# kazuto1011/dusty-gan-v2

Hardware: AMD Instinct MI355X
Metric: range-images/sec (G+D step) on dusty_v2 64x512 (higher is better)
Workload: dtype bf16; 1 GPU; configs[2]: configs/gans/dusty_v2.yaml full G+D train step (G step + D step + lazy R1 + ADA + EMA + Adam), 64x512 synthetic; global_batch=64, per_gpu_batch=64, parallelism=dp1, hip_graph=True, d_epilogue_dtype=fp32, pe_table_precomputed=True

## Files before the change

dusty-gan-v2_amd/csrc/api.hip:

```cpp
#include "common.h"

extern "C" int dgv2_abi_version(void) { return 48; }
```

dusty-gan-v2_amd/csrc/fir_mfma.hip:

```cpp
#include <type_traits>

#include "gemm_core.h"

namespace {

constexpr int FM_CT = 32;
constexpr int FM_CB = 32;
constexpr int FM_WIN = FM_CT + 16;
#ifndef DGV2_FIR_RS
#define DGV2_FIR_RS 8
#endif
constexpr int FM_RS = DGV2_FIR_RS;
constexpr int FM_RING = 2 * FM_RS;
static_assert(FM_RS == 8 || FM_RS == 4, "rows per step");
constexpr int FM_XBYTES = FM_RS * FM_WIN * 64;
constexpr int FM_ZROW = 2048 + 64;
constexpr int FM_ZBYTES = FM_RING * FM_ZROW;
constexpr int FM_YROW = 2048 + 16;
constexpr int FM_YBYTES = FM_RS * FM_YROW;
constexpr int FM_NLD = FM_RS * FM_WIN * 4 / 256;

struct FMGeom {
  int B, C, H, W, nt;
  const uint4* bands;
  const bf16_t* ref;
  float alpha, ascale;
  float* partial;
  uint8_t* y8;
};

struct FMTabs {
  int H, W, Eh, Ew;
  const int* idx_h; const float* coef_h; const int* cnt_h;
  const int* idx_w; const float* coef_w; const int* cnt_w;
  int* err;
};

typedef __attribute__((ext_vector_type(4))) unsigned fm_u32x4;
typedef __attribute__((address_space(3))) s16x4 fm_lds_s16x4;

__device__ __forceinline__ unsigned fm_pack2(float a, float b) {
  union { bf16_t h[2]; unsigned u; } p;
  p.h[0] = (bf16_t)a;
  p.h[1] = (bf16_t)b;
  return p.u;
}

__global__ __launch_bounds__(64) void fir_bands_kernel(uint4* __restrict__ bands, FMTabs t) {
  const int lane = threadIdx.x, li = lane & 15, kg = lane >> 4;
  const int nh = t.H / FM_RS + 1;
  float v[8];
#pragma unroll
  for (int j = 0; j < 8; ++j) v[j] = 0.f;
  bool bad = false;
  if ((int)blockIdx.x < nh) {
    const int s = blockIdx.x, ho = s * FM_RS - FM_RS / 2 + li;
    if (li < FM_RS && ho >= 0 && ho < t.H) {
      const int n = t.cnt_h[ho];
      for (int e = 0; e < n; ++e) {
        const int r = t.idx_h[ho * t.Eh + e];
        const float cf = t.coef_h[ho * t.Eh + e];
        if (r < s * FM_RS - FM_RS || r >= s * FM_RS + FM_RS || r < 0 || r >= t.H) bad = true;
#pragma unroll
        for (int j = 0; j < 8; ++j)
          if ((r & (FM_RING - 1)) == 8 * kg + j) v[j] += cf;
      }
    }
  } else {
    const int wt = blockIdx.x - nh, wo = 16 * wt + li;
    const int n = t.cnt_w[wo];
    for (int e = 0; e < n; ++e) {
      int rel = t.idx_w[wo * t.Ew + e] - (16 * wt - 8);
      rel = rel < 0 ? rel + t.W : (rel >= t.W ? rel - t.W : rel);
      const float cf = t.coef_w[wo * t.Ew + e];
      if ((unsigned)rel >= 32u) bad = true;
#pragma unroll
      for (int j = 0; j < 8; ++j)
        if (rel == 8 * kg + j) v[j] += cf;
    }
  }
#pragma unroll
  for (int j = 0; j < 8; ++j)
    if ((float)(bf16_t)v[j] != v[j]) bad = true;
  bands[(int64_t)blockIdx.x * 64 + lane] =
      make_uint4(fm_pack2(v[0], v[1]), fm_pack2(v[2], v[3]), fm_pack2(v[4], v[5]), fm_pack2(v[6], v[7]));
  if (bad) atomicOr(t.err, DGV2_STATUS_FIR_TABLE);
}

// ... 150 lines not shown
          bsum[j] += o.get(j);
        }
      }
      if constexpr (!ACT) {
        if (g.y8) {
          float f[8];
#pragma unroll
          for (int j = 0; j < 8; ++j) f[j] = o.get(j);
          *reinterpret_cast<uint2*>(g.y8 + off) = pack_fp8x8(f);
          continue;
        }
      }
      if (g.nt) o.store_nt(y + off);
      else o.store(y + off);
    }
    th = th_next;
  }

  if constexpr (ACT) {
    float* fold = reinterpret_cast<float*>(Xs);
    __syncthreads();
#pragma unroll
    for (int j = 0; j < 8; ++j) fold[tid * 8 + j] = bsum[j];
    __syncthreads();
    if (tid < FM_CB) {
      const int o8 = tid >> 3, j = tid & 7;
      float s2 = 0.f;
      for (int t = o8; t < 256; t += 4) s2 += fold[t * 8 + j];
      g.partial[((int64_t)b * gridDim.x + c0col / FM_CT) * g.C + cb0 + tid] = s2;
    }
  }
}

__global__ __launch_bounds__(256) void fm_bias_reduce_kernel(float* __restrict__ gb, const float* __restrict__ partial,
                                                             int nblk, int C) {
  __shared__ float red[16];
  const int c = blockIdx.x;
  float s = 0.f;
#pragma unroll 4
  for (int k = threadIdx.x; k < nblk; k += 256) s += partial[(int64_t)k * C + c];
  s = block_sum(s, red);
  if (threadIdx.x == 0) gb[c] = s;
}

bool fm_covers(int B, int C, int H, int W) {
  return B > 0 && C % FM_CB == 0 && H % FM_RS == 0 && H >= FM_RS && W % FM_CT == 0 && W >= FM_CT && B < 65536 &&
         C / FM_CB < 65536;
}

constexpr size_t FM_LDS = (size_t)FM_XBYTES + FM_ZBYTES + FM_YBYTES;

int64_t fm_band_bytes(int H, int W) { return 1024 * ((int64_t)H / FM_RS + 1 + W / 16); }

}

extern "C" int dgv2_fir_same_mfma_prep(void* bands, int64_t bands_bytes, int64_t* bytes_needed, const int* idx_h,
                                       const float* coef_h, const int* cnt_h, int Eh, const int* idx_w, const float* coef_w,
                                       const int* cnt_w, int Ew, int H, int W, int* status, void* stream) {
  if (H < FM_RS || H % FM_RS || W < FM_CT || W % FM_CT || Eh < 1 || Ew < 1) return DGV2_ENOTSUP;
  const int64_t need = fm_band_bytes(H, W);
  if (bytes_needed) *bytes_needed = need;
  if (!bands) return bytes_needed ? 0 : DGV2_EINVAL;
  if (bands_bytes < need || !aligned16(bands) || !idx_h || !coef_h || !cnt_h || !idx_w || !coef_w || !cnt_w) return DGV2_EINVAL;
  if (!status) return DGV2_EINVAL;
  FMTabs t{H, W, Eh, Ew, idx_h, coef_h, cnt_h, idx_w, coef_w, cnt_w, status};
  fir_bands_kernel<<<(int)(need / 1024), 64, 0, (hipStream_t)stream>>>((uint4*)bands, t);
  DGV2_RETURN_LAST();
}

extern "C" int dgv2_fir_same_mfma(void* y, const void* x, const void* bands, int B, int C, int H, int W, void* stream) {
  if (!y || !x || !bands) return DGV2_EINVAL;
  if (!fm_covers(B, C, H, W)) return DGV2_ENOTSUP;
  if (!aligned16(x) || !aligned16(y) || !aligned16(bands)) return DGV2_EINVAL;
  FMGeom g{B, C, H, W, nt_output((int64_t)B * H * W * C * 2) ? 1 : 0, (const uint4*)bands, nullptr, 1.f, 1.f, nullptr, nullptr};
  auto kern = fir_same_mfma_kernel<false>;
  if (FM_LDS > 64 * 1024) {
    hipError_t e = hipFuncSetAttribute((const void*)kern, hipFuncAttributeMaxDynamicSharedMemorySize, (int)FM_LDS);
    if (e != hipSuccess) return (int)e;
  }
  kern<<<dim3(W / FM_CT, C / FM_CB, B), 256, FM_LDS, (hipStream_t)stream>>>((bf16_t*)y, (const bf16_t*)x, g);
  DGV2_RETURN_LAST();
}

extern "C" int dgv2_fir_same_mfma_q8(void* y8, const void* x, const void* bands, int B, int C, int H, int W, void* stream) {
  if (!y8 || !x || !bands) return DGV2_EINVAL;
  if (!fm_covers(B, C, H, W)) return DGV2_ENOTSUP;
  if (!aligned16(x) || (reinterpret_cast<uintptr_t>(y8) & 7) || !aligned16(bands)) return DGV2_EINVAL;
  FMGeom g{B, C, H, W, 0, (const uint4*)bands, nullptr, 1.f, 1.f, nullptr, (uint8_t*)y8};
  auto kern = fir_same_mfma_kernel<false>;
  if (FM_LDS > 64 * 1024) {
    hipError_t e = hipFuncSetAttribute((const void*)kern, hipFuncAttributeMaxDynamicSharedMemorySize, (int)FM_LDS);
    if (e != hipSuccess) return (int)e;
  }
  kern<<<dim3(W / FM_CT, C / FM_CB, B), 256, FM_LDS, (hipStream_t)stream>>>((bf16_t*)nullptr, (const bf16_t*)x, g);
  DGV2_RETURN_LAST();
}

extern "C" int dgv2_fir_same_mfma_actbwd(void* y, float* gb, float* scratch, int64_t scratch_elems, int64_t* blocks_needed,
                                         const void* x, const void* ref, const void* bands, int B, int C, int H, int W,
                                         float alpha, float scale, void* stream) {
  if (!fm_covers(B, C, H, W)) return DGV2_ENOTSUP;
  const int64_t blocks = (int64_t)B * (W / FM_CT);
  if (blocks_needed) *blocks_needed = blocks;
  if (!scratch) return blocks_needed ? 0 : DGV2_EINVAL;
  if (!y || !gb || !x || !ref || !bands) return DGV2_EINVAL;
  if (scratch_elems < blocks * C || !aligned16(x) || !aligned16(y) || !aligned16(ref) || !aligned16(bands)) return DGV2_EINVAL;
  FMGeom g{B, C, H, W, 0, (const uint4*)bands, (const bf16_t*)ref, alpha, scale, scratch, nullptr};
  auto kern = fir_same_mfma_kernel<true>;
  if (FM_LDS > 64 * 1024) {
    hipError_t e = hipFuncSetAttribute((const void*)kern, hipFuncAttributeMaxDynamicSharedMemorySize, (int)FM_LDS);
    if (e != hipSuccess) return (int)e;
  }
  hipStream_t st = (hipStream_t)stream;
  kern<<<dim3(W / FM_CT, C / FM_CB, B), 256, FM_LDS, st>>>((bf16_t*)y, (const bf16_t*)x, g);
  fm_bias_reduce_kernel<<<C, 256, 0, st>>>(gb, scratch, (int)blocks, C);
  DGV2_RETURN_LAST();
}
```

dusty-gan-v2_amd/dgv2_native/__init__.py:

```python
import ctypes
import os

import torch

_HERE = os.path.dirname(os.path.abspath(__file__))
LIB_PATH = os.environ.get("DGV2_LIB_PATH") or os.path.join(os.path.dirname(_HERE), "lib", "libdgv2.so")

F32, BF16 = 0, 1
ABI_VERSION = 48

_c_int, _c_i64, _c_f32, _c_ptr = ctypes.c_int, ctypes.c_int64, ctypes.c_float, ctypes.c_void_p

SIGNATURES = {
    "dgv2_abi_version": [],
    "dgv2_fused_bias_act": [_c_ptr] * 4 + [_c_i64] * 3 + [_c_int, _c_int, _c_f32, _c_f32, _c_int, _c_ptr],
    "dgv2_bias_grad": [_c_ptr, _c_ptr, _c_i64, _c_i64, _c_i64, _c_int, _c_ptr],
    "dgv2_bias_act_bwd": [_c_ptr] * 4 + [_c_i64, _c_int, _c_f32, _c_f32, _c_ptr, _c_i64, _c_int, _c_ptr],
    "dgv2_bias_act_bwd_rs": [_c_ptr] * 4 + [_c_i64, _c_int, _c_f32, _c_f32, _c_ptr, _c_ptr, _c_i64, _c_int, _c_ptr],
    "dgv2_surface_normal": [_c_ptr, _c_ptr] + [_c_int] * 5 + [_c_ptr],
    "dgv2_mbstd_cat_fwd": [_c_ptr] * 3 + [_c_int] * 7 + [_c_ptr],
    "dgv2_mbstd_cat_bwd": [_c_ptr] * 3 + [_c_int] * 7 + [_c_ptr],
    "dgv2_gemm_x3": [_c_ptr, _c_ptr, _c_i64, _c_ptr, _c_ptr, _c_int, _c_int, _c_i64, _c_int, _c_int, _c_i64, _c_i64, _c_i64,
                     _c_int, _c_f32, _c_ptr],
    "dgv2_pe_wgrad_scratch": [_c_ptr] + [_c_int] * 4,
    "dgv2_pe_wgrad": [_c_ptr, _c_ptr, _c_i64, _c_ptr, _c_ptr] + [_c_int] * 4 + [_c_i64, _c_int, _c_ptr],
    "dgv2_mbstd_cat_fwd_x": [_c_ptr] * 3 + [_c_int] * 8 + [_c_ptr],
    "dgv2_mbstd_cat_bwd_x": [_c_ptr] * 3 + [_c_int] * 8 + [_c_ptr],
    "dgv2_scale_cast": [_c_ptr] * 3 + [_c_i64, _c_int, _c_int, _c_int, _c_ptr],
    "dgv2_upfirdn2d": [_c_ptr] * 3 + [_c_int] * 15 + [_c_ptr],
    "dgv2_resample": [_c_ptr] * 4 + [_c_int] * 19 + [_c_ptr],
    "dgv2_resample_tab": [_c_ptr] * 5 + [_c_int] + [_c_ptr] * 3 + [_c_int] * 10 + [_c_ptr],
    "dgv2_resample_tab_add": [_c_ptr] * 6 + [_c_int] + [_c_ptr] * 3 + [_c_int] * 8 + [_c_ptr],
    "dgv2_resample_tab_add_affine": [_c_ptr] * 8 + [_c_int] + [_c_ptr] * 3 + [_c_int] * 8 + [_c_ptr],
    "dgv2_fourier_feature": [_c_ptr] * 5 + [_c_int] * 8 + [_c_ptr],
    "dgv2_downsample_angle": [_c_ptr] * 4 + [_c_int] * 5 + [_c_ptr],
    "dgv2_bmm_nn": [_c_ptr] * 3 + [_c_int] * 6 + [_c_i64, _c_ptr, _c_int, _c_f32, _c_f32, _c_int, _c_int, _c_ptr],
    "dgv2_bmm_tn": [_c_ptr] * 3 + [_c_int] * 7 + [_c_ptr],
    "dgv2_bmm_nn_cat": [_c_ptr] * 4 + [_c_int] * 5 + [_c_ptr, _c_int, _c_f32, _c_f32, _c_int, _c_int, _c_ptr],
    "dgv2_bmm_nn_cat_sq": [_c_ptr] * 4 + [_c_int] * 5 + [_c_ptr, _c_ptr, _c_int, _c_f32, _c_f32, _c_int, _c_int, _c_ptr, _c_int, _c_ptr,
                           _c_ptr],
    "dgv2_bmm_nn_sq": [_c_ptr] * 3 + [_c_int] * 6 + [_c_i64, _c_ptr, _c_ptr, _c_int, _c_f32, _c_f32, _c_ptr, _c_int, _c_int, _c_ptr, _c_int,
                       _c_ptr, _c_ptr],
# ... 6 lines not shown
    "dgv2_kitti_project": [_c_ptr] * 4 + [_c_int] * 4 + [_c_f32, _c_f32, _c_int, _c_ptr],
    "dgv2_fps_scratch": [_c_ptr, _c_int, _c_int],
    "dgv2_fps": [_c_ptr] * 3 + [_c_int] * 3 + [_c_ptr],
    "dgv2_gather_points": [_c_ptr] * 3 + [_c_int] * 4 + [_c_ptr],
    "dgv2_gather_points_grad": [_c_ptr] * 3 + [_c_int] * 4 + [_c_ptr],
    "dgv2_chamfer_fwd": [_c_ptr] * 6 + [_c_int] * 3 + [_c_ptr],
    "dgv2_nn_search": [_c_ptr] * 4 + [_c_int] * 4 + [_c_ptr],
    "dgv2_chamfer_bwd": [_c_ptr] * 8 + [_c_int] * 3 + [_c_ptr],
    "dgv2_emd_approxmatch": [_c_ptr] * 4 + [_c_int] * 3 + [_c_ptr],
    "dgv2_emd_matchcost": [_c_ptr] * 4 + [_c_int] * 3 + [_c_ptr],
    "dgv2_emd_matchcost_grad": [_c_ptr] * 5 + [_c_int] * 3 + [_c_ptr],
    "dgv2_nsgan_loss": [_c_ptr, _c_ptr, _c_ptr, _c_int, _c_int, _c_f32, _c_ptr, _c_ptr, _c_ptr],
    "dgv2_modconv_pe_dgrad_actbwd": [_c_ptr, _c_ptr, _c_ptr, _c_i64] + [_c_ptr] * 5 + [_c_f32, _c_f32] + [_c_int] * 4 + [_c_ptr],
    "dgv2_colmean_lerp": [_c_ptr, _c_ptr, _c_int, _c_int, _c_i64, _c_f32, _c_ptr],
    "dgv2_d_tail_fwd": [_c_ptr] * 6 + [_c_int, _c_int] + [_c_f32] * 4 + [_c_ptr],
    "dgv2_d_tail_bwd": [_c_ptr] * 7 + [_c_int, _c_int] + [_c_f32] * 4 + [_c_ptr],
    "dgv2_rng_fill": [_c_ptr] * 5 + [_c_int, _c_ptr, _c_ptr],
    "dgv2_modconv_up_fwd": [_c_ptr] * 4 + [_c_int] * 7 + [_c_ptr] * 6 + [_c_int, _c_f32, _c_f32, _c_int, _c_ptr, _c_int, _c_ptr,
                            _c_ptr],
    "dgv2_modconv_up_t_lag": [_c_ptr] * 4 + [_c_f32] + [_c_ptr] * 4 + [_c_int] * 9 + [_c_ptr, _c_int, _c_ptr, _c_ptr],
    "dgv2_fir_same_mfma_q8": [_c_ptr] * 3 + [_c_int] * 4 + [_c_ptr],
    "dgv2_resample_tab_q8": [_c_ptr] * 5 + [_c_int] + [_c_ptr] * 3 + [_c_int] * 7 + [_c_ptr],
    "dgv2_fp8_quant_weights": [_c_ptr] * 6 + [_c_int] + [_c_ptr] * 3,
    "dgv2_fp8_dequant": [_c_ptr, _c_ptr, _c_i64, _c_f32, _c_ptr],
    "dgv2_conv_taps_fp8": [_c_ptr] * 4 + [_c_int] * 14 + [_c_ptr, _c_int, _c_ptr, _c_ptr, _c_int, _c_f32, _c_f32, _c_ptr],
    "dgv2_modconv_up_t": [_c_ptr] * 5 + [_c_f32] + [_c_int] * 9 + [_c_ptr],
    "dgv2_up2_lag_sumsq": [_c_ptr] * 5 + [_c_int] * 5 + [_c_ptr, _c_int, _c_ptr, _c_ptr],
    "dgv2_resample_tab_actbwd": [_c_ptr, _c_ptr, _c_ptr, _c_i64, _c_ptr, _c_ptr, _c_ptr] + [_c_ptr] * 3 + [_c_int] + [_c_ptr] * 3
                                + [_c_int] * 7 + [_c_f32, _c_f32, _c_int, _c_ptr],
    "dgv2_fir_same_mfma_prep": [_c_ptr, _c_i64, _c_ptr] + [_c_ptr] * 3 + [_c_int] + [_c_ptr] * 3 + [_c_int] * 3 + [_c_ptr, _c_ptr],
    "dgv2_fir_same_mfma": [_c_ptr] * 3 + [_c_int] * 4 + [_c_ptr],
    "dgv2_fir_same_mfma_actbwd": [_c_ptr, _c_ptr, _c_ptr, _c_i64, _c_ptr, _c_ptr, _c_ptr, _c_ptr] + [_c_int] * 4
                                 + [_c_f32, _c_f32, _c_ptr],
    "dgv2_resample_tab_sq": [_c_ptr] * 5 + [_c_int] + [_c_ptr] * 3 + [_c_int] * 10 + [_c_ptr, _c_int, _c_ptr, _c_ptr],
    "dgv2_bmm_tn_cat": [_c_ptr] * 4 + [_c_int] * 6 + [_c_ptr],
    "dgv2_lerp_list": [_c_ptr] * 3 + [_c_int, _c_f32, _c_ptr],
    "dgv2_adam_prep": [_c_ptr, _c_ptr, _c_f32, _c_f32, _c_ptr],
    "dgv2_adam_step": [_c_ptr] * 5 + [_c_int, _c_ptr] + [_c_f32] * 4 + [_c_ptr],
    "dgv2_pack2d": [_c_ptr] * 4 + [_c_int] * 3 + [_c_ptr],
    "dgv2_unpack2d": [_c_ptr] * 4 + [_c_int] * 3 + [_c_ptr],
    "dgv2_ema_scalar": [_c_ptr] * 3 + [_c_int] + [_c_f32] * 3 + [_c_int, _c_ptr, _c_int, _c_ptr],
    "dgv2_ema_scalar_group": [_c_ptr, _c_ptr, _c_int, _c_ptr, _c_int] + [_c_f32] * 3 + [_c_int, _c_ptr, _c_ptr],
    "dgv2_bmm_nn_small": [_c_ptr] * 4 + [_c_int] * 5 + [_c_ptr],
    "dgv2_bmm_nn_small_act": [_c_ptr] * 4 + [_c_int] * 4 + [_c_ptr, _c_ptr, _c_f32, _c_f32, _c_ptr, _c_ptr, _c_i64, _c_ptr, _c_int,
                              _c_ptr],
    "dgv2_bmm_tn_small": [_c_ptr] * 3 + [_c_int] * 5 + [_c_ptr],
    "dgv2_head_bwd": [_c_ptr] * 5 + [_c_i64] + [_c_ptr] * 7 + [_c_f32, _c_f32] + [_c_int] * 5 + [_c_ptr],
    "dgv2_transpose_list": [_c_ptr] * 5 + [_c_int] * 3 + [_c_ptr],
    "dgv2_mod_prep_all_fwd": [_c_ptr] * 13 + [_c_ptr, _c_int, _c_int, _c_ptr],
    "dgv2_mod_prep_all_bwd": [_c_ptr, _c_i64] + [_c_ptr] * 15 + [_c_ptr, _c_int, _c_int, _c_ptr, _c_i64, _c_ptr],
    "dgv2_mod_prep_all_bwd_scratch": [_c_ptr, _c_ptr, _c_ptr, _c_int, _c_int],
    "dgv2_mod_prep_fwd": [_c_ptr] * 8 + [_c_int] * 9 + [_c_ptr],
    "dgv2_mod_prep_bwd": [_c_ptr] * 11 + [_c_int] * 9 + [_c_ptr],
    "dgv2_sum_squares": [_c_ptr, _c_ptr, _c_i64, _c_int, _c_int, _c_int, _c_ptr],
    "dgv2_conv_fwd": [_c_ptr] * 3 + [_c_int] * 10 + [_c_ptr, _c_int, _c_f32, _c_f32, _c_int, _c_ptr],
    "dgv2_conv_taps": [_c_ptr] * 3 + [_c_int] * 17 + [_c_ptr] + [_c_int] * 3 + [_c_ptr, _c_ptr, _c_int, _c_f32, _c_f32, _c_int,
                                                                               _c_ptr],
    "dgv2_conv_taps_ex": [_c_ptr] * 3 + [_c_int] * 14 + [_c_ptr, _c_int, _c_int, _c_ptr, _c_int, _c_ptr] + [_c_int] * 3
    + [_c_ptr, _c_ptr, _c_int, _c_f32, _c_f32, _c_int, _c_ptr],
    "dgv2_conv_taps_ld": [_c_ptr, _c_int, _c_ptr, _c_ptr] + [_c_int] * 14 + [_c_ptr, _c_int, _c_int, _c_ptr, _c_int, _c_ptr] + [_c_int] * 3
    + [_c_ptr, _c_ptr, _c_int, _c_f32, _c_f32, _c_int, _c_ptr],
    "dgv2_conv_wgrad_direct": [_c_ptr] * 3 + [_c_int] * 10 + [_c_ptr],
    "dgv2_bmm_tn_stream_scratch": [_c_ptr] + [_c_int] * 6,
    "dgv2_bmm_tn_stream": [_c_ptr, _c_ptr, _c_i64, _c_ptr, _c_ptr] + [_c_int] * 6 + [_c_ptr],
    "dgv2_bmm_tn_stream_x": [_c_ptr, _c_ptr, _c_i64, _c_ptr, _c_ptr] + [_c_int] * 7 + [_c_ptr],
    "dgv2_bmm_tn_stream_ld": [_c_ptr, _c_i64, _c_ptr, _c_i64, _c_ptr, _c_ptr] + [_c_int] * 7 + [_c_ptr],
# ... 139 lines not shown
```

dusty-gan-v2_amd/gans/models/ops/native/act_resample.py:

```python
import contextlib
import math
import os

import torch
from torch.autograd import Function

import dgv2_native as N


_EPS_U = torch.finfo(torch.float32).eps


def _dt(t):
    return N.dtype_code(t)


def _bias_act_raw(x, bias, ref, grad, alpha, scale, step_b, size_b):
    N.check(x, bias, ref)
    y = torch.empty_like(x)
    N.call("dgv2_fused_bias_act", N.ptr(y), N.ptr(x), N.ptr(bias), N.ptr(ref), x.numel(), step_b, size_b,
           3, grad, alpha, scale, _dt(x), N.stream())
    return y


# ... 145 lines not shown
        key = (H, W, bool(adjoint), str(device))
        if key not in self._tab:
            Ho, Wo = self.out_size(H, W)
            tabs = []
            for L, Lo, taps, (k, u, d, p0, _), wrap in zip((H, W), (Ho, Wo), self.taps_cpu, self.axes,
                                                           (False, self.ring)):
                idx, coef, cnt, E = self._axis_rows(L, Lo, taps.tolist(), k, u, d, p0, wrap, adjoint)
                tabs.append((idx.to(device), coef.to(device), cnt.to(device), E))
            self._tab[key] = tabs
            ok = (Ho, Wo) == (H, W)
            for axis, (L, (k, u, d, p0, _), wrap, taps) in enumerate(zip((H, W), self.axes, (False, self.ring), self.taps_cpu)):
                if not ok:
                    break
                idx, coef, cnt, E = self._axis_rows(L, L, taps.tolist(), k, u, d, p0, wrap, adjoint)
                o = torch.arange(L, dtype=torch.int32)[:, None]
                live = torch.arange(E)[None, :] < cnt[:, None]
                dense = torch.zeros(L, L).index_put_((o.expand(L, E)[live].long(), idx[live].long()), coef[live], accumulate=True)
                ok = ok and E <= 6 and L <= (128 if axis == 0 else 1 << 20) and bool((dense == dense.bfloat16().float()).all())
                if axis == 0:
                    ok = ok and bool(((idx - o).abs()[live] <= 4).all())
                else:
                    ok = ok and bool((((idx - o + 8) % L)[live] < 24).all())
            self._mfma[key] = ok
        return self._tab[key]

    def mfma_ok(self, H, W, adjoint, device):
        self.tables(H, W, adjoint, device)
        return self._mfma[(H, W, bool(adjoint), str(device))]

    def bands(self, H, W, adjoint, device):
        key = (H, W, bool(adjoint), str(device), "bands")
        if key not in self._tab:
            self._tab[key] = None
            if H >= _FIR_MFMA_MIN_H and H % 8 == 0 and W % 32 == 0 and self.mfma_ok(H, W, adjoint, device):
                (ih, chh, nh, Eh), (iw, cw, nw, Ew) = self.tables(H, W, adjoint, device)
                need = _ct.c_int64(0)
                tabs = (N.ptr(ih), N.ptr(chh), N.ptr(nh), Eh, N.ptr(iw), N.ptr(cw), N.ptr(nw), Ew, H, W,
                        N.ptr(N.status_word(device)))
                if N.try_call("dgv2_fir_same_mfma_prep", None, 0, _ct.addressof(need), *tabs, N.stream()):
                    buf = torch.empty(need.value, device=device, dtype=torch.uint8)
                    N.call("dgv2_fir_same_mfma_prep", N.ptr(buf), buf.numel(), None, *tabs, N.stream())
                    self._tab[key] = buf
        return self._tab[key]


_SQ_CAP = 8192


_FUSED_SQ = os.environ.get("DGV2_NO_FUSED_SUMSQ") is None


_FIR_MFMA = os.environ.get("DGV2_NO_FIR_MFMA") is None
_FIR_MFMA_MIN_H = int(os.environ.get("DGV2_FIR_MFMA_MIN_H", "32"))


def _sq_args(dev):
    return torch.empty(_SQ_CAP, device=dev, dtype=torch.float32), _ct.c_int(0)


def _resample_raw(x, spec, adjoint, in_hw, out=None, ldy=None, ldx=None, C=None, sq=None):
    B = x.shape[0]
    H, W = in_hw
    Ho, Wo = spec.out_size(H, W)
    ldx = x.shape[3] if ldx is None else ldx
    C = ldx if C is None else C
    ih, iw = (Ho, Wo) if adjoint else (H, W)
    oh, ow = (H, W) if adjoint else (Ho, Wo)
    if out is None:
        out = torch.empty((B, oh, ow, C), device=x.device, dtype=x.dtype)
        ldy = C
    (ih_idx, ih_coef, ih_cnt, Eh), (iw_idx, iw_coef, iw_cnt, Ew) = spec.tables(H, W, adjoint, x.device)
    if (_FIR_MFMA and sq is None and x.dtype == torch.bfloat16 and ldx == C and ldy == C and (ih, iw) == (oh, ow)
            and C % 32 == 0):
        bands = spec.bands(H, W, adjoint, x.device)
        if bands is not None and N.try_call("dgv2_fir_same_mfma", N.ptr(out), N.ptr(x), N.ptr(bands), B, C, oh, ow, N.stream()):
            return out
    if sq is not None:
        N.call("dgv2_resample_tab_sq", N.ptr(out), N.ptr(x), N.ptr(ih_idx), N.ptr(ih_coef), N.ptr(ih_cnt), Eh,
               N.ptr(iw_idx), N.ptr(iw_coef), N.ptr(iw_cnt), Ew, B, C, ldx, ldy, ih, iw, oh, ow, _dt(x), N.ptr(sq[0]),
               _SQ_CAP, _ct.addressof(sq[1]), N.stream())
        return out
    N.call("dgv2_resample_tab", N.ptr(out), N.ptr(x), N.ptr(ih_idx), N.ptr(ih_coef), N.ptr(ih_cnt), Eh,
           N.ptr(iw_idx), N.ptr(iw_coef), N.ptr(iw_cnt), Ew, B, C, ldx, ldy, ih, iw, oh, ow, _dt(x), N.stream())
    return out


class _ResampleSq(Function):

    @staticmethod
    def forward(ctx, x, spec, in_hw):
        ctx.set_materialize_grads(False)
        x = x.contiguous()
        N.check(x)
        ctx.cfg = (spec, in_hw)
        sq = _sq_args(x.device)
        y = _resample_raw(x, spec, False, in_hw, sq=sq)
        part = sq[0][:sq[1].value] if sq[1].value > 0 else sum_squares(y)
        ctx.mark_non_differentiable(part)
        return y, part

    @staticmethod
    def backward(ctx, g, _):
        spec, in_hw = ctx.cfg
        return (None if g is None else _Resample.apply(g, spec, True, in_hw)), None, None


def resample_sq(x, spec):
    if not _FUSED_SQ:
# ... 88 lines not shown
```

dusty-gan-v2_amd/gans/models/ops/native/conv.py:

```python
import contextlib
import os
from typing import NamedTuple, Optional

import torch
from torch.autograd import Function

import dgv2_native as N
from . import act_resample as _act_resample
from .act_resample import *
from .modgemm import *


class ConvGeom:
    def __init__(self, kh, kw, stride, pad, ring):
        self.kh, self.kw, self.stride, self.pad, self.ring = kh, kw, stride, pad, int(bool(ring))

    def out_hw(self, H, W):
        return (H + 2 * self.pad - self.kh) // self.stride + 1, (W + 2 * self.pad - self.kw) // self.stride + 1

    @property
    def ring3x3(self):
        return bool(self.ring) and (self.kh, self.kw, self.pad) == (3, 3, 1)


# ... 759 lines not shown
            w8ts[-1]._dgv2_clive = int(c)
        off += n
        off8 += m8 if f else 0
        off8t += m8t if ft else 0
    srcs = [p.detach() for p, _, _ in entries]
    N.check(*srcs)
    rest = (_ptr_array(srcs), _int_array([d[0] for d in dims]), _int_array([d[1] for d in dims]),
            _int_array([d[2] for d in dims]), _int_array([d[3] for d in dims]),
            (_ct.c_float * L)(*[float(s) for _, s, _ in entries]), L, N.dtype_code(flat_f), N.stream())
    if image8 is None:
        N.call("dgv2_conv_weight_bank", _ptr_array(wfs), _ptr_array(wts), *rest)
        return list(zip(wfs, wts))
    N.call("dgv2_conv_weight_bank_ex", _ptr_array(wfs), _ptr_array(wts), _ptr_array(w8s), _ptr_array(w8ts), *rest)
    return list(zip(wfs, wts, w8s, w8ts))


_ACTBWD_BLOCKS = {}


_FUSED_ACTBWD = os.environ.get("DGV2_NO_FUSED_ACTBWD") is None


def _resample_actbwd(g, out, spec, in_hw, alpha, scale):
    if not _FUSED_ACTBWD or g.dtype != out.dtype:
        return None
    B, H, W, C = out.shape
    Ho, Wo = spec.out_size(H, W)
    (ih_idx, ih_coef, ih_cnt, Eh), (iw_idx, iw_coef, iw_cnt, Ew) = spec.tables(H, W, True, g.device)
    tabs = (N.ptr(ih_idx), N.ptr(ih_coef), N.ptr(ih_cnt), Eh, N.ptr(iw_idx), N.ptr(iw_coef), N.ptr(iw_cnt), Ew)
    bands = None
    if _act_resample._FIR_MFMA and g.dtype == torch.bfloat16 and (Ho, Wo) == (H, W) and C % 32 == 0:
        bands = spec.bands(H, W, True, g.device)
    mfma = bands is not None
    entry = "dgv2_fir_same_mfma_actbwd" if mfma else "dgv2_resample_tab_actbwd"
    tabs = (N.ptr(bands),) if mfma else tabs
    geo = (B, C, H, W) if mfma else (B, C, Ho, Wo, H, W)
    tail = (alpha, scale) if mfma else (alpha, scale, _dt(g))
    key = (entry, B, H, W, C, Eh, Ew, _dt(g))
    if key not in _ACTBWD_BLOCKS:
        nb = _ct.c_int64(0)
        ok = N.try_call(entry, None, None, None, 0, _ct.addressof(nb), None, None, *tabs, *geo, *tail, N.stream())
        _ACTBWD_BLOCKS[key] = nb.value if ok else 0
    nblk = _ACTBWD_BLOCKS[key]
    if nblk == 0:
        return None
    g = g.contiguous()
    N.check(g, out)
    gpre = torch.empty_like(out)
    gb = torch.empty(C, device=g.device, dtype=torch.float32)
    scratch = torch.empty(nblk * C, device=g.device, dtype=torch.float32)
    N.call(entry, N.ptr(gpre), N.ptr(gb), N.ptr(scratch), scratch.numel(), None, N.ptr(g), N.ptr(out), *tabs, *geo, *tail,
           N.stream())
    return gpre, gb


class _Conv(Function):

    @staticmethod
    def forward(ctx, x, w, bias, resid, x8, ep):
        ctx.set_materialize_grads(False)
        assert (ep.act is not None) == (bias is not None) and ep.resid == (resid is not None) and not (ep.act and ep.resid)
        assert ep.act is not None or (ep.down is None and not ep.fork), "blur/down and fork belong to the activation's forms"
        assert ep.fp8 is None or (ep.down is None and not ep.fork), "an e4m3 input has no blur/down or fork form"
        alpha, scale = ep.act or (0.2, 1.0)
        act = 0 if ep.act is None else 3
        if bias is not None:
            ctx.size_b = bias.numel()
            bias = bias.detach().float().contiguous()
        if resid is not None:
            resid = resid.contiguous()
        if ep.fp8 is not None:
# ... 80 lines not shown
```

include/dgv2.h:

```cpp
#ifndef DGV2_H
#define DGV2_H

#include <stdint.h>

#ifdef __cplusplus
extern "C" {
#endif

#define DGV2_F32 0
#define DGV2_BF16 1
#define DGV2_FP8 2
#define DGV2_EINVAL (-1)
#define DGV2_ENOTSUP (-3)

#define DGV2_STATUS_X_INEXACT 1
#define DGV2_STATUS_FIR_TABLE 2

int dgv2_abi_version(void);

int dgv2_fused_bias_act(void* y, const void* x, const void* bias, const void* ref,
                        int64_t size_x, int64_t step_b, int64_t size_b,
                        int act, int grad, float alpha, float scale, int dtype, void* stream);

int dgv2_bias_grad(float* gb, const void* x, int64_t size_x, int64_t step_b, int64_t size_b,
// ... 20 lines not shown
                  int ring, int adjoint, int dtype, void* stream);

int dgv2_resample_tab(void* y, const void* x, const int* idx_h, const float* coef_h, const int* cnt_h,
                      int Eh, const int* idx_w, const float* coef_w, const int* cnt_w, int Ew,
                      int B, int C, int ldx, int ldy, int in_h, int in_w, int out_h, int out_w,
                      int dtype, void* stream);

int dgv2_resample_tab_add(void* y, const void* x, const void* resid, const int* idx_h, const float* coef_h,
                          const int* cnt_h, int Eh, const int* idx_w, const float* coef_w, const int* cnt_w, int Ew,
                          int B, int C, int in_h, int in_w, int out_h, int out_w, int dtype, void* stream);
int dgv2_resample_tab_add_affine(void* y, const void* x, const void* resid, const float* rscale, const float* rbias,
                                 const int* idx_h, const float* coef_h, const int* cnt_h, int Eh, const int* idx_w,
                                 const float* coef_w, const int* cnt_w, int Ew, int B, int C, int in_h, int in_w, int out_h,
                                 int out_w, int dtype, void* stream);

int dgv2_resample_tab_sq(void* y, const void* x, const int* idx_h, const float* coef_h, const int* cnt_h,
                         int Eh, const int* idx_w, const float* coef_w, const int* cnt_w, int Ew,
                         int B, int C, int ldx, int ldy, int in_h, int in_w, int out_h, int out_w,
                         int dtype, float* sumsq, int sumsq_cap, int* sumsq_used, void* stream);

int dgv2_resample_tab_actbwd(void* y, float* gb, float* scratch, int64_t scratch_elems, int64_t* blocks_needed,
                             const void* x, const void* ref, const int* idx_h, const float* coef_h,
                             const int* cnt_h, int Eh, const int* idx_w, const float* coef_w, const int* cnt_w,
                             int Ew, int B, int C, int in_h, int in_w, int out_h, int out_w, float alpha,
                             float scale, int dtype, void* stream);

int dgv2_fir_same_mfma_prep(void* bands, int64_t bands_bytes, int64_t* bytes_needed, const int* idx_h, const float* coef_h,
                            const int* cnt_h, int Eh, const int* idx_w, const float* coef_w, const int* cnt_w, int Ew,
                            int H, int W, int* status, void* stream);
int dgv2_fir_same_mfma(void* y, const void* x, const void* bands, int B, int C, int H, int W, void* stream);
int dgv2_fir_same_mfma_actbwd(void* y, float* gb, float* scratch, int64_t scratch_elems, int64_t* blocks_needed,
                              const void* x, const void* ref, const void* bands, int B, int C, int H, int W, float alpha,
                              float scale, void* stream);

int dgv2_fourier_feature(void* out, const float* angle, const float* shift,
                         const float* freqs, const float* phase,
                         int B, int Ba, int H, int W, int F, int ld, int c0, int dtype, void* stream);

int dgv2_downsample_angle(float* out, const float* in, const float* shift, const float* taps,
                          int B, int Ba, int H, int W, int ring, void* stream);

int dgv2_bmm_nn(void* y, const void* x, const void* w, int B, int P, int I, int O,
                int ldx, int ldy, int64_t wstride, const float* bias, int act, float alpha, float scale,
                int dtype, int ydtype, void* stream);
int dgv2_bmm_tn(float* gw, const void* gy, const void* x, int B, int P, int I, int O,
                int ldgy, int ldx, int dtype, void* stream);

int dgv2_bmm_nn_cat(void* y, const void* xa, const void* xs, const void* w, int B, int P, int Ka, int Ks,
                    int O, const float* bias, int act, float alpha, float scale, int dtype, int ydtype,
                    void* stream);
int dgv2_modconv_up_fwd(void* y, const void* t, const void* xs, const void* wimg, int B, int Hout, int Wout, int Hin,
                        int Win, int Ks, int O, const int* idx_h, const float* coef_h, const int* idx_w,
                        const float* coef_w, const float* bias, const float* in_scale, int act, float alpha, float scale,
                        int dtype, float* sumsq, int sumsq_cap, int* sumsq_used, void* stream);
int dgv2_modconv_up_t(void* tcm, void* wimg, const void* h, const void* w, const float* row_scale, float gain, int B,
                      int Hlow, int Wlow, int Ka, int Ks, int O, int I, int koff, int dtype, void* stream);
int dgv2_modconv_up_t_lag(void* tcm, void* wimg, const void* h, const void* w, float gain, const float* ghd,
                          const float* gho, const float* gwd, const float* gwo, int B, int Hlow, int Wlow, int Ka, int Ks,
                          int O, int I, int koff, int dtype, float* sumsq, int sumsq_cap, int* sumsq_used, void* stream);
int dgv2_up2_lag_sumsq(const void* h, const float* ghd, const float* gho, const float* gwd, const float* gwo, int B,
                       int Hin, int Win, int C, int dtype, float* sumsq, int sumsq_cap, int* sumsq_used, void* stream);
int dgv2_bmm_nn_sq(void* y, const void* x, const void* w, int B, int P, int I, int O, int ldx, int ldy,
                   int64_t wstride, const float* row_scale, const float* bias, int act, float alpha, float scale,
                   const void* resid , int dtype, int ydtype,
                   float* sumsq, int sumsq_cap, int* sumsq_used, void* stream);
int dgv2_bmm_nn_cat_sq(void* y, const void* xa, const void* xs, const void* w, int B, int P, int Ka, int Ks,
// ... 266 lines not shown
```

Measured before the change: 5488 range-images/s.

## Add whole-image MFMA FIR kernel for 8- and 16-row feature maps

Adds a new FIR resampling kernel for small-height maps (H=8 or 16). Each block holds the full image height and filters both vertically and horizontally with MFMA, looping over several images with a double-buffered register prefetch. A full-height band matrix is built in the prep kernel. Dispatch now routes these small maps, which previously used the generic table resampler, to the new kernel by default, including the fused activation-backward path. This trades extra band setup and larger LDS use (lower occupancy at H=16) for tensor-core throughput on the low-resolution layers.

Result: no change. 5516 range-images/s (median of 6 runs) (+0.5%).

```diff
diff --git a/dusty-gan-v2_amd/csrc/api.hip b/dusty-gan-v2_amd/csrc/api.hip
--- a/dusty-gan-v2_amd/csrc/api.hip
+++ b/dusty-gan-v2_amd/csrc/api.hip
@@ -1,3 +1,3 @@
 #include "common.h"
 
-extern "C" int dgv2_abi_version(void) { return 48; }
+extern "C" int dgv2_abi_version(void) { return 49; }
diff --git a/dusty-gan-v2_amd/csrc/fir_mfma.hip b/dusty-gan-v2_amd/csrc/fir_mfma.hip
--- a/dusty-gan-v2_amd/csrc/fir_mfma.hip
+++ b/dusty-gan-v2_amd/csrc/fir_mfma.hip
@@ -1,3 +1,4 @@
+#include <algorithm>
 #include <type_traits>
 
 #include "gemm_core.h"
@@ -27,6 +28,9 @@
   float alpha, ascale;
   float* partial;
   uint8_t* y8;
+#ifdef DGV2_ABLATE
+  int ablate;
+#endif
 };
 
 struct FMTabs {
@@ -53,7 +57,19 @@
 #pragma unroll
   for (int j = 0; j < 8; ++j) v[j] = 0.f;
   bool bad = false;
-  if ((int)blockIdx.x < nh) {
+  if ((int)blockIdx.x == nh + t.W / 16) {
+    if (li < t.H) {
+      const int n = t.cnt_h[li];
+      for (int e = 0; e < n; ++e) {
+        const int r = t.idx_h[li * t.Eh + e];
+        const float cf = t.coef_h[li * t.Eh + e];
+        if (r < 0 || r >= t.H) bad = true;
+#pragma unroll
+        for (int j = 0; j < 8; ++j)
+          if (r == 8 * kg + j) v[j] += cf;
+      }
+    }
+  } else if ((int)blockIdx.x < nh) {
     const int s = blockIdx.x, ho = s * FM_RS - FM_RS / 2 + li;
     if (li < FM_RS && ho >= 0 && ho < t.H) {
       const int n = t.cnt_h[ho];
@@ -270,6 +286,220 @@
   }
 }
 
+template <int HH>
+struct FI {
+  static constexpr int XBYTES = HH * FM_WIN * 64;
+  static constexpr int ZBYTES = HH * FM_ZROW;
+  static constexpr int YBYTES = HH * FM_YROW;
+  static constexpr int NLD = HH * FM_WIN * 4 / 256;
+  static constexpr size_t LDS = (size_t)XBYTES + ZBYTES + YBYTES;
+};
+
+template <int HH, bool ACT>
+__global__ __launch_bounds__(256, HH == 8 ? 2 : 1) void fir_img_mfma_kernel(bf16_t* __restrict__ y, const bf16_t* __restrict__ x,
+                                                                           FMGeom g, int per) {
+  using K = FI<HH>;
+  extern __shared__ __attribute__((aligned(16))) unsigned char smem[];
+  unsigned char* Xs = smem;
+  unsigned char* Zs = Xs + K::XBYTES;
+  unsigned char* Ys = Zs + K::ZBYTES;
+  const int tid = threadIdx.x, wave = tid >> 6, lane = tid & 63;
+  const int li = lane & 15, kg = lane >> 4;
+  const int q = li >> 2, p = li & 3;
+  int vid = blockIdx.x + gridDim.x * (blockIdx.y + gridDim.y * blockIdx.z);
+  {
+    const int nblk = gridDim.x * gridDim.y * gridDim.z;
+    if ((nblk & 7) == 0) vid = (vid & 7) * (nblk >> 3) + (vid >> 3);
+  }
+  const int c0col = (vid % (int)gridDim.x) * FM_CT;
+  const int cb0 = ((vid / (int)gridDim.x) % (int)gridDim.y) * FM_CB;
+  const int chunk = vid / (int)(gridDim.x * gridDim.y);
+  const int b0 = chunk * per, b1 = min(b0 + per, g.B);
+  const int64_t imgsz = (int64_t)HH * g.W * g.C;
+
+  const int nh = HH / FM_RS + 1;
+  uint4 tw[2];
+  tw[0] = g.bands[(int64_t)(nh + c0col / 16) * 64 + lane];
+  tw[1] = g.bands[(int64_t)(nh + 1 + c0col / 16) * 64 + lane];
+  const uint4 th = g.bands[(int64_t)(nh + g.W / 16) * 64 + lane];
+
+  int goff[K::NLD];
+  int xoff[K::NLD];
+#pragma unroll
+  for (int i = 0; i < K::NLD; ++i) {
+    const int id = tid + 256 * i;
+    const int o8 = id & 3, j = (id >> 2) % FM_WIN, r = id / (4 * FM_WIN);
+    int gc = c0col - 8 + j;
+    gc = gc < 0 ? gc + g.W : (gc >= g.W ? gc - g.W : gc);
+    goff[i] = (r * g.W + gc) * g.C + cb0 + o8 * 8;
+    xoff[i] = ((r * FM_WIN + j) * 4 + (o8 ^ (((j >> 3) & 1) << 1))) * 16;
+  }
+  fm_u32x4 rg[K::NLD];
+  auto issue = [&](int b) {
+#pragma unroll
+    for (int i = 0; i < K::NLD; ++i) {
+#ifdef DGV2_ABLATE
+      if (g.ablate & 4) { rg[i] = (fm_u32x4){(unsigned)b, 0u, 0u, 0u}; continue; }
+#endif
+      rg[i] = *reinterpret_cast<const fm_u32x4*>(x + b * imgsz + goff[i]);
+    }
+  };
+  auto commit = [&]() {
+#pragma unroll
+    for (int i = 0; i < K::NLD; ++i) *reinterpret_cast<fm_u32x4*>(Xs + xoff[i]) = rg[i];
+  };
+  issue(b0);
+  commit();
+  if (b0 + 1 < b1) issue(b0 + 1);
+  __syncthreads();
+
+  float bsum[8];
+#pragma unroll
+  for (int j = 0; j < 8; ++j) bsum[j] = 0.f;
+
+  for (int b = b0; b < b1; ++b) {
+    const int64_t img = b * imgsz;
+    {
+      uint4 af[HH];
+#pragma unroll
+      for (int job = 0; job < HH; ++job) {
+        const int rr = job >> 2, ct = (job >> 1) & 1, wt = job & 1;
+        const int r = (HH / 4) * wave + rr;
+        const int j = 16 * wt + 8 * kg + q;
+        const int o8 = (2 * ct + (p >> 1)) ^ ((kg & 1) << 1);
+        const unsigned char* a0 = Xs + ((r * FM_WIN + j) * 4 + o8) * 16 + (p & 1) * 8;
+        union { uint4 u; s16x4 h[2]; } a;
+        a.h[0] = __builtin_amdgcn_ds_read_tr16_b64_v4i16((fm_lds_s16x4*)a0);
+        a.h[1] = __builtin_amdgcn_ds_read_tr16_b64_v4i16((fm_lds_s16x4*)(a0 + 4 * 64));
+        af[job] = a.u;
+      }
+      f32x4 acc[HH];
+#pragma unroll
+      for (int job = 0; job < HH; ++job) {
+        acc[job] = (f32x4){0.f, 0.f, 0.f, 0.f};
+#ifdef DGV2_ABLATE
+        if (g.ablate & 2) { acc[job][0] = __uint_as_float(af[job].x); continue; }
+#endif
+        Mfma16<bf16_t>::run(acc[job], af[job], tw[job & 1]);
+      }
+#pragma unroll
+      for (int job = 0; job < HH; ++job) {
+        const int rr = job >> 2, ct = (job >> 1) & 1, wt = job & 1;
+        const int slot = (HH / 4) * wave + rr;
+        const int wp = 16 * wt + li;
+        const int u = (4 * ct + kg) ^ ((wp >> 2) & 7) ^ ((slot >> 3) << 2);
+        uint2 pk = make_uint2(fm_pack2(acc[job][0], acc[job][1]), fm_pack2(acc[job][2], acc[job][3]));
+        *reinterpret_cast<uint2*>(Zs + slot * FM_ZROW + wp * 64 + u * 8) = pk;
+      }
+    }
+    __syncthreads();
+    if (b + 1 < b1) commit();
+    if (b + 2 < b1) issue(b + 2);
+    vec16<bf16_t> fref[HH / 2];
+    if constexpr (ACT) {
+#pragma unroll
+      for (int i = 0; i < HH / 2; ++i) {
+        const int id = tid + 256 * i;
+        fref[i].load(g.ref + img + ((int64_t)(id >> 7) * g.W + c0col + ((id >> 2) & 31)) * g.C + cb0 + (id & 3) * 8);
+      }
+    }
+
+    {
+      uint4 af[16];
+#pragma unroll
+      for (int job = 0; job < 16; ++job) {
+        const int wp = 8 * wave + (job >> 1), ct = job & 1;
+        const int hi = HH == 16 ? (kg & 1) : 0;
+        const int slot = 8 * hi + q;
+        const int u = (4 * ct + p) ^ ((wp >> 2) & 7) ^ (hi << 2);
+        const unsigned char* a0 = Zs + slot * FM_ZROW + wp * 64 + u * 8;
+        union { uint4 u4; s16x4 h[2]; } a;
+        a.h[0] = __builtin_amdgcn_ds_read_tr16_b64_v4i16((fm_lds_s16x4*)a0);
+        a.h[1] = __builtin_amdgcn_ds_read_tr16_b64_v4i16((fm_lds_s16x4*)(a0 + 4 * FM_ZROW));
+        af[job] = a.u4;
+      }
+      f32x4 acc[16];
+#pragma unroll
+      for (int job = 0; job < 16; ++job) {
+        acc[job] = (f32x4){0.f, 0.f, 0.f, 0.f};
+#ifdef DGV2_ABLATE
+        if (g.ablate & 2) { acc[job][0] = __uint_as_float(af[job].x); continue; }
+#endif
+        Mfma16<bf16_t>::run(acc[job], af[job], th);
+      }
+      if (li < HH) {
+#pragma unroll
+        for (int job = 0; job < 16; ++job) {
+          const int wp = 8 * wave + (job >> 1), ct = job & 1;
+          uint2 pk = make_uint2(fm_pack2(acc[job][0], acc[job][1]), fm_pack2(acc[job][2], acc[job][3]));
+          *reinterpret_cast<uint2*>(Ys + li * FM_YROW + wp * 64 + (4 * ct + kg) * 8) = pk;
+        }
+      }
+    }
+    __syncthreads();
+
+#pragma unroll
+    for (int i = 0; i < HH / 2; ++i) {
+      const int id = tid + 256 * i;
+      const int o8 = id & 3, px = (id >> 2) & 31, n = id >> 7;
+      vec16<bf16_t> o;
+      o.raw = *reinterpret_cast<const uint4*>(Ys + n * FM_YROW + px * 64 + o8 * 16);
+      const int64_t off = img + ((int64_t)n * g.W + c0col + px) * g.C + cb0 + o8 * 8;
+      if constexpr (ACT) {
+#pragma unroll
+        for (int j = 0; j < 8; ++j) {
+          const float a = o.get(j);
+          o.set(j, (fref[i].get(j) > 0.f ? a : a * g.alpha) * g.ascale);
+          bsum[j] += o.get(j);
+        }
+      }
+#ifdef DGV2_ABLATE
+      if ((g.ablate & 1) && o.raw.x != 0x7fc1u) continue;
+#endif
+      if (g.nt) o.store_nt(y + off);
+      else o.store(y + off);
+    }
+  }
+
+  if constexpr (ACT) {
+    float* fold = reinterpret_cast<float*>(Xs);
+    __syncthreads();
+#pragma unroll
+    for (int j = 0; j < 8; ++j) fold[tid * 8 + j] = bsum[j];
+    __syncthreads();
+    if (tid < FM_CB) {
+      const int o8 = tid >> 3, j = tid & 7;
+      float s2 = 0.f;
+      for (int t = o8; t < 256; t += 4) s2 += fold[t * 8 + j];
+      g.partial[((int64_t)chunk * gridDim.x + c0col / FM_CT) * g.C + cb0 + tid] = s2;
+    }
+  }
+}
+
+int fi_per(int B, int C, int H, int W, int asked) {
+  if (asked > 0) return std::min(asked, B);
+  const int tiles = (W / FM_CT) * (C / FM_CB), want = H == 8 ? 512 : 256;
+  const int chunks = std::min(B, std::max(1, want / tiles));
+  return (B + chunks - 1) / chunks;
+}
+
+template <int HH, bool ACT>
+int fi_launch(bf16_t* y, const bf16_t* x, const FMGeom& g, int per, hipStream_t st) {
+  auto kern = fir_img_mfma_kernel<HH, ACT>;
+  if (FI<HH>::LDS > 64 * 1024) {
+    hipError_t e = hipFuncSetAttribute((const void*)kern, hipFuncAttributeMaxDynamicSharedMemorySize, (int)FI<HH>::LDS);
+    if (e != hipSuccess) return (int)e;
+  }
+#ifdef DGV2_ABLATE
+  FMGeom ga = g;
+  ga.ablate = getenv("DGV2_FI_ABLATE") ? atoi(getenv("DGV2_FI_ABLATE")) : 0;
+  kern<<<dim3(g.W / FM_CT, g.C / FM_CB, (g.B + per - 1) / per), 256, FI<HH>::LDS, st>>>(y, x, ga, per);
+  return 0;
+#endif
+  kern<<<dim3(g.W / FM_CT, g.C / FM_CB, (g.B + per - 1) / per), 256, FI<HH>::LDS, st>>>(y, x, g, per);
+  return 0;
+}
+
 __global__ __launch_bounds__(256) void fm_bias_reduce_kernel(float* __restrict__ gb, const float* __restrict__ partial,
                                                              int nblk, int C) {
   __shared__ float red[16];
@@ -288,7 +518,9 @@
 
 constexpr size_t FM_LDS = (size_t)FM_XBYTES + FM_ZBYTES + FM_YBYTES;
 
-int64_t fm_band_bytes(int H, int W) { return 1024 * ((int64_t)H / FM_RS + 1 + W / 16); }
+bool fm_img_rows(int H) { return H == 8 || H == 16; }
+
+int64_t fm_band_bytes(int H, int W) { return 1024 * ((int64_t)H / FM_RS + 1 + W / 16 + (fm_img_rows(H) ? 1 : 0)); }
 
 }
 
@@ -354,3 +586,36 @@
   fm_bias_reduce_kernel<<<C, 256, 0, st>>>(gb, scratch, (int)blocks, C);
   DGV2_RETURN_LAST();
 }
+
+
+extern "C" int dgv2_fir_img_mfma(void* y, const void* x, const void* bands, int B, int C, int H, int W, int images_per_block,
+                                 void* stream) {
+  if (!y || !x || !bands) return DGV2_EINVAL;
+  if (!fm_img_rows(H) || !fm_covers(B, C, H, W)) return DGV2_ENOTSUP;
+  if (!aligned16(x) || !aligned16(y) || !aligned16(bands)) return DGV2_EINVAL;
+  FMGeom g{B, C, H, W, nt_output((int64_t)B * H * W * C * 2) ? 1 : 0, (const uint4*)bands, nullptr, 1.f, 1.f, nullptr, nullptr};
+  const int per = fi_per(B, C, H, W, images_per_block);
+  const int rc = H == 8 ? fi_launch<8, false>((bf16_t*)y, (const bf16_t*)x, g, per, (hipStream_t)stream)
+                        : fi_launch<16, false>((bf16_t*)y, (const bf16_t*)x, g, per, (hipStream_t)stream);
+  if (rc) return rc;
+  DGV2_RETURN_LAST();
+}
+
+extern "C" int dgv2_fir_img_mfma_actbwd(void* y, float* gb, float* scratch, int64_t scratch_elems, int64_t* blocks_needed,
+                                        const void* x, const void* ref, const void* bands, int B, int C, int H, int W,
+                                        float alpha, float scale, int images_per_block, void* stream) {
+  if (!fm_img_rows(H) || !fm_covers(B, C, H, W)) return DGV2_ENOTSUP;
+  const int per = fi_per(B, C, H, W, images_per_block);
+  const int64_t blocks = (int64_t)((B + per - 1) / per) * (W / FM_CT);
+  if (blocks_needed) *blocks_needed = blocks;
+  if (!scratch) return blocks_needed ? 0 : DGV2_EINVAL;
+  if (!y || !gb || !x || !ref || !bands) return DGV2_EINVAL;
+  if (scratch_elems < blocks * C || !aligned16(x) || !aligned16(y) || !aligned16(ref) || !aligned16(bands)) return DGV2_EINVAL;
+  FMGeom g{B, C, H, W, 0, (const uint4*)bands, (const bf16_t*)ref, alpha, scale, scratch, nullptr};
+  hipStream_t st = (hipStream_t)stream;
+  const int rc = H == 8 ? fi_launch<8, true>((bf16_t*)y, (const bf16_t*)x, g, per, st)
+                        : fi_launch<16, true>((bf16_t*)y, (const bf16_t*)x, g, per, st);
+  if (rc) return rc;
+  fm_bias_reduce_kernel<<<C, 256, 0, st>>>(gb, scratch, (int)blocks, C);
+  DGV2_RETURN_LAST();
+}
diff --git a/dusty-gan-v2_amd/dgv2_native/__init__.py b/dusty-gan-v2_amd/dgv2_native/__init__.py
--- a/dusty-gan-v2_amd/dgv2_native/__init__.py
+++ b/dusty-gan-v2_amd/dgv2_native/__init__.py
@@ -7,7 +7,7 @@
 LIB_PATH = os.environ.get("DGV2_LIB_PATH") or os.path.join(os.path.dirname(_HERE), "lib", "libdgv2.so")
 
 F32, BF16 = 0, 1
-ABI_VERSION = 48
+ABI_VERSION = 49
 
 _c_int, _c_i64, _c_f32, _c_ptr = ctypes.c_int, ctypes.c_int64, ctypes.c_float, ctypes.c_void_p
 
@@ -80,6 +80,9 @@
     "dgv2_fir_same_mfma": [_c_ptr] * 3 + [_c_int] * 4 + [_c_ptr],
     "dgv2_fir_same_mfma_actbwd": [_c_ptr, _c_ptr, _c_ptr, _c_i64, _c_ptr, _c_ptr, _c_ptr, _c_ptr] + [_c_int] * 4
                                  + [_c_f32, _c_f32, _c_ptr],
+    "dgv2_fir_img_mfma": [_c_ptr] * 3 + [_c_int] * 5 + [_c_ptr],
+    "dgv2_fir_img_mfma_actbwd": [_c_ptr, _c_ptr, _c_ptr, _c_i64, _c_ptr, _c_ptr, _c_ptr, _c_ptr] + [_c_int] * 4
+                                + [_c_f32, _c_f32, _c_int, _c_ptr],
     "dgv2_resample_tab_sq": [_c_ptr] * 5 + [_c_int] + [_c_ptr] * 3 + [_c_int] * 10 + [_c_ptr, _c_int, _c_ptr, _c_ptr],
     "dgv2_bmm_tn_cat": [_c_ptr] * 4 + [_c_int] * 6 + [_c_ptr],
     "dgv2_lerp_list": [_c_ptr] * 3 + [_c_int, _c_f32, _c_ptr],
diff --git a/dusty-gan-v2_amd/gans/models/ops/native/act_resample.py b/dusty-gan-v2_amd/gans/models/ops/native/act_resample.py
--- a/dusty-gan-v2_amd/gans/models/ops/native/act_resample.py
+++ b/dusty-gan-v2_amd/gans/models/ops/native/act_resample.py
@@ -201,7 +201,7 @@
         key = (H, W, bool(adjoint), str(device), "bands")
         if key not in self._tab:
             self._tab[key] = None
-            if H >= _FIR_MFMA_MIN_H and H % 8 == 0 and W % 32 == 0 and self.mfma_ok(H, W, adjoint, device):
+            if _fir_mfma_entry(H) is not None and H % 8 == 0 and W % 32 == 0 and self.mfma_ok(H, W, adjoint, device):
                 (ih, chh, nh, Eh), (iw, cw, nw, Ew) = self.tables(H, W, adjoint, device)
                 need = _ct.c_int64(0)
                 tabs = (N.ptr(ih), N.ptr(chh), N.ptr(nh), Eh, N.ptr(iw), N.ptr(cw), N.ptr(nw), Ew, H, W,
@@ -221,6 +221,14 @@
 
 _FIR_MFMA = os.environ.get("DGV2_NO_FIR_MFMA") is None
 _FIR_MFMA_MIN_H = int(os.environ.get("DGV2_FIR_MFMA_MIN_H", "32"))
+_FIR_IMG_H = frozenset(int(h) for h in os.environ.get("DGV2_FIR_IMG_H", "8,16").split(",") if h)
+_FIR_IMG_PER = 0
+
+
+def _fir_mfma_entry(H):
+    if H in _FIR_IMG_H:
+        return "dgv2_fir_img_mfma"
+    return "dgv2_fir_same_mfma" if H >= _FIR_MFMA_MIN_H else None
 
 
 def _sq_args(dev):
@@ -242,7 +250,9 @@
     if (_FIR_MFMA and sq is None and x.dtype == torch.bfloat16 and ldx == C and ldy == C and (ih, iw) == (oh, ow)
             and C % 32 == 0):
         bands = spec.bands(H, W, adjoint, x.device)
-        if bands is not None and N.try_call("dgv2_fir_same_mfma", N.ptr(out), N.ptr(x), N.ptr(bands), B, C, oh, ow, N.stream()):
+        entry = _fir_mfma_entry(oh)
+        per = (_FIR_IMG_PER,) if entry == "dgv2_fir_img_mfma" else ()
+        if bands is not None and N.try_call(entry, N.ptr(out), N.ptr(x), N.ptr(bands), B, C, oh, ow, *per, N.stream()):
             return out
     if sq is not None:
         N.call("dgv2_resample_tab_sq", N.ptr(out), N.ptr(x), N.ptr(ih_idx), N.ptr(ih_coef), N.ptr(ih_cnt), Eh,
diff --git a/dusty-gan-v2_amd/gans/models/ops/native/conv.py b/dusty-gan-v2_amd/gans/models/ops/native/conv.py
--- a/dusty-gan-v2_amd/gans/models/ops/native/conv.py
+++ b/dusty-gan-v2_amd/gans/models/ops/native/conv.py
@@ -815,11 +815,13 @@
     if _act_resample._FIR_MFMA and g.dtype == torch.bfloat16 and (Ho, Wo) == (H, W) and C % 32 == 0:
         bands = spec.bands(H, W, True, g.device)
     mfma = bands is not None
-    entry = "dgv2_fir_same_mfma_actbwd" if mfma else "dgv2_resample_tab_actbwd"
+    entry = _act_resample._fir_mfma_entry(H) + "_actbwd" if mfma else "dgv2_resample_tab_actbwd"
     tabs = (N.ptr(bands),) if mfma else tabs
     geo = (B, C, H, W) if mfma else (B, C, Ho, Wo, H, W)
     tail = (alpha, scale) if mfma else (alpha, scale, _dt(g))
-    key = (entry, B, H, W, C, Eh, Ew, _dt(g))
+    if entry == "dgv2_fir_img_mfma_actbwd":
+        tail += (_act_resample._FIR_IMG_PER,)
+    key = (entry, B, H, W, C, Eh, Ew, _dt(g), tail[2:])
     if key not in _ACTBWD_BLOCKS:
         nb = _ct.c_int64(0)
         ok = N.try_call(entry, None, None, None, 0, _ct.addressof(nb), None, None, *tabs, *geo, *tail, N.stream())
diff --git a/include/dgv2.h b/include/dgv2.h
--- a/include/dgv2.h
+++ b/include/dgv2.h
@@ -76,6 +76,11 @@
 int dgv2_fir_same_mfma_actbwd(void* y, float* gb, float* scratch, int64_t scratch_elems, int64_t* blocks_needed,
                               const void* x, const void* ref, const void* bands, int B, int C, int H, int W, float alpha,
                               float scale, void* stream);
+int dgv2_fir_img_mfma(void* y, const void* x, const void* bands, int B, int C, int H, int W, int images_per_block,
+                      void* stream);
+int dgv2_fir_img_mfma_actbwd(void* y, float* gb, float* scratch, int64_t scratch_elems, int64_t* blocks_needed,
+                             const void* x, const void* ref, const void* bands, int B, int C, int H, int W, float alpha,
+                             float scale, int images_per_block, void* stream);
 
 int dgv2_fourier_feature(void* out, const float* angle, const float* shift,
                          const float* freqs, const float* phase,
```
